# Martinsos/edlib

Hardware: NVIDIA H100
Metric: GCUPS (higher is better)
Workload: dtype u32

## Files before the change

__graft_entry__.py:

```python
import os
import subprocess
import sys

REPO = os.path.dirname(os.path.abspath(__file__))
sys.path.insert(0, REPO)


def build():
    subprocess.run(["make", "-C", os.path.join(REPO, "edlib_b200", "csrc")], check=True)
    subprocess.run(["make", "-C", os.path.join(REPO, "oracle"), "liboracle.so"], check=True)
    subprocess.run(["make", "-C", os.path.join(REPO, "oracle"), "ref"], check=True)
    subprocess.run(["make", "-C", os.path.join(REPO, "tests", "emul")], check=True)
    subprocess.run(["make", "-C", os.path.join(REPO, "tests", "kernel_probe")], check=True)
    subprocess.run(["make", "-C", os.path.join(REPO, "oracle"), "reftests"], check=True)
    subprocess.run(["make", "-C", os.path.join(REPO, "oracle"), "pybinding"], check=True)
    import edlib_b200
    import ctypes
    ctypes.CDLL(os.path.join(REPO, "edlib_b200", "lib", "libedlib_b200.so"))


def smoke():
    sys.path.insert(0, os.path.join(REPO, "tests"))
    from edlib_b200 import workloads
    from edlib_b200._ffi import EdlibLib, product_path
    lib = EdlibLib(product_path(), has_batch=True)
    assert lib.lib.edlibB200Available() == 1, "no CUDA device / kernels: the product has no CPU path"
    oracle = EdlibLib(os.path.join(REPO, "oracle", "liboracle.so"), prefix="oracle")
    target, reads = workloads.reads_vs_target(num_reads=512, read_len=150, target_len=100_000, seed=3)
# ... 16 lines not shown
```

edlib_b200/csrc/eb_common.h:

```cpp
#pragma once
#include <stdint.h>

#if defined(__CUDACC__)
#define EB_HD __host__ __device__ __forceinline__
#define EB_D __device__ __forceinline__
#else
#define EB_HD inline
#define EB_D inline
#endif

namespace eb {

struct U2 { uint32_t x, y; };

constexpr int KPOS = 4;

struct Rec {
    int best;
    int cnt;
    int last;
    int rsv;
    int pos[KPOS];
};

// ... 28 lines not shown
    int ncodes;
    const uint8_t* eqtab;
    int chunks;
    int chunkLen;
    int halo;
    Rec* recs;
    Ovf* ovf;
    int* ovfCount;
    int ovfCap;
    int prefixLen;
    int rangeMode;
};

struct K1WParams {
    const uint8_t* tcodes;
    const uint8_t* qcodes;
    const uint64_t* qoff;
    const int* qlen;
    const int* readList;
    const int* kInit;
    const int* winStart;
    const int* winLen;
    const int* trackFrom;
    int numReads;
    const int* countPtr;
    int checkAfter;
    int ncodes;
    const uint8_t* eqtab;
    WinRec* recs;
    Ovf* ovf;
    int* ovfCount;
    int ovfCap;
};

struct LJob {
    uint64_t qOff;
    uint64_t tOff;
    uint64_t matOff;
    int m, n;
    int kInit;
    int trackFrom;
};
struct LParams {
// ... 43 lines not shown
    U2* mat;
    int* colOut;
    Rec* recs;
    Ovf* ovf;
    int* ovfCount;
    int ovfCap;
};

struct PeqParams {
    const WJob* jobs;
    int numJobs;
    const uint8_t* qcodes;
    uint32_t* peq;
    int ncodes;
    const uint8_t* eqtab;
};

struct TbJob {
    uint64_t matOff;
    uint64_t qOff;
    uint64_t peqOff;
    uint64_t tOff;
    uint64_t outOff;
    int m, n, nWp;
    int rsv;
};
struct TbParams {
    const TbJob* jobs;
    int numJobs;
    const U2* mat;
// ... 72 lines not shown
    const int* qlen;
    const int* readList;
    int firstPair;
    const int* thr;
    int kBound, seedK;
    int numReads;
    int maxLen;
    int Ls;
    int Lidx, sigma, numKeys;
    const int* bucketStart;
    const int* positions;
    int maxBucket;
    int level;
    int spread;
    int* winPair;
    int* winK;
    int* winStart;
    int* winLen;
    int* winTf;
    int winCap;
    int* winCount;
    SeedPlan* plan;
};
struct Leftover {
    int pair;
    int excl;
    int bound;
};
enum RecState : int { REC_DONE = 100, REC_PENDING = 101 };
struct WinReduceParams {
// ... 172 lines not shown
```

edlib_b200/csrc/eb_core.h:

```cpp
#pragma once
#include <type_traits>

#include "eb_common.h"

#if defined(__CUDA_ARCH__)
#define EB_UNROLL _Pragma("unroll")
#else
#define EB_UNROLL
#endif

namespace eb {


EB_HD uint32_t funnel_l1(uint32_t lo, uint32_t hi) {
#if defined(__CUDA_ARCH__)
    return __funnelshift_l(lo, hi, 1);
#else
    return (hi << 1) | (lo >> 31);
#endif
}

EB_HD int popcount32(uint32_t v) {
#if defined(__CUDA_ARCH__)
    return __popc(v);
// ... 584 lines not shown
            EB_UNROLL
            for (int q = 0; q < 16; ++q) b.template column<false>(j + q, (cur.w[q >> 2] >> (8 * (q & 3))) & 255u);
        }
        for (; j + 15 <= hi; j += 16) {
            const Sym16 cur = v;
            if (j + 31 <= hi) v = load_sym16(tsyms + j + 16);
            EB_UNROLL
            for (int q = 0; q < 16; ++q) b.template column<true>(j + q, (cur.w[q >> 2] >> (8 * (q & 3))) & 255u);
        }
    }
    for (; j <= hi; ++j) b.template column<true>(j, tsyms[j]);
    bestIo = b.best;
    cntIo = b.cnt;
}

template <int NW, class WAcc>
EB_HD void k1w_profile(const K1WParams& p, int pair, int m, WAcc& acc) {
    for (int code = 0; code < p.ncodes; ++code) {
        acc.store_word(code, 0, ~0u);
        acc.store_word(code, 1, ~0u);
        acc.store_word(code, NW + 2, 0u);
        acc.store_word(code, NW + 3, 0u);
    }
    K1View<NW, WAcc> k1acc{acc};
    k1_build_peq<NW>(k1acc, p.qcodes + p.qoff[pair], m, MODE_HW, p.ncodes, p.eqtab);
}
template <int NW, class WAcc>
EB_HD void k1w_thread(const K1WParams& p, int slot, WAcc& acc) {
    const int pair = p.readList[slot];
    const int m = p.qlen[pair];
    WinRec* rec = p.recs + slot;
    k1w_profile<NW>(p, pair, m, acc);
    K1View<NW, WAcc> k1acc{acc};
    const int ws = p.winStart[slot], tf = p.trackFrom[slot], len = p.winLen[slot];
    const int kInit = p.kInit[slot];
    const int t = kInit - 1;
    const int hi = len - 1;
    if (t >= 0 && (hi - tf) + 2 * t + 1 <= 64) {
        const int c0 = tf - (m + t) > 0 ? tf - (m + t) : 0;
        int best = kInit, cnt = 0;
        k1b_sweep(acc, p.tcodes + ws, ws, m, 32 * NW - m, c0, tf, hi, t, p.checkAfter, best, cnt, rec, p, slot);
        rec->best = best;
        rec->cnt = cnt;
        return;
    }
    K1State<NW> st;
    k1_init<NW>(st, m, kInit);
// ... 2 lines not shown
        const int cntj = tf - j < 32 ? tf - j : 32;
        k1_columns<NW, false, false>(st, k1acc, PtrSyms{p.tcodes + ws + j}, cntj, ws + j, rec, slot, nullptr, nullptr, 0);
        if (st.up - st.down - (len - (j + cntj)) >= st.best) {
            hopeless = true;
            break;
        }
    }
    if (!hopeless)
        k1_columns<NW, false, true>(st, k1acc, PtrSyms{p.tcodes + ws + tf}, len - tf, ws + tf, rec, slot, p.ovf, p.ovfCount, p.ovfCap);
    rec->best = st.best;
    rec->cnt = st.cnt;
}

template <int NW, class WAcc>
EB_HD void k1w_hits_thread(const K1WParams& p, const HitParams& h, int slot, WAcc& acc) {
    HitSink sink;
    if (!hit_sink_open(h, slot, sink)) return;
    const int pair = p.readList[slot];
    const int m = p.qlen[pair];
    k1w_profile<NW>(p, pair, m, acc);
    K1View<NW, WAcc> k1acc{acc};
    const int ws = p.winStart[slot], tf = p.trackFrom[slot], len = p.winLen[slot];
    const int t = p.kInit[slot] - 1;
    const int hi = len - 1;
    if (t >= 0 && (hi - tf) + 2 * t + 1 <= 64) {
        const int c0 = tf - (m + t) > 0 ? tf - (m + t) : 0;
        int best = t, cnt = 0;
        k1b_sweep(acc, p.tcodes + ws, ws, m, 32 * NW - m, c0, tf, hi, t, p.checkAfter, best, cnt, &sink, p, slot);
    } else {
        K1State<NW> st;
        k1_init<NW>(st, m, t);
        bool hopeless = false;
        for (int j = 0; j < tf; j += 32) {
            const int cntj = tf - j < 32 ? tf - j : 32;
            k1_columns<NW, false, false>(st, k1acc, PtrSyms{p.tcodes + ws + j}, cntj, ws + j, &sink, slot, nullptr, nullptr, 0);
// ... 78 lines not shown
        }
        int lo = first - t, hi = last + t;
        if (lo <= prevHi) lo = prevHi + 1;
        if (lo < 0) lo = 0;
        if (hi > p.n - 1) hi = p.n - 1;
        if (lo > hi) continue;
        prevHi = hi;
        int ws = lo - (m + t);
        if (ws < 0) ws = 0;
        ws &= ~15;
        f(nW, ws, lo, hi);
        ++nW;
    }
    return nW;
}
EB_HD void seed_window_store(const SeedPlanParams& p, int w, int pair, int t, int ws, int lo, int hi) {
    p.winPair[w] = pair;
    p.winK[w] = t + 1;
    p.winStart[w] = ws;
    p.winLen[w] = hi - ws + 1;
    p.winTf[w] = lo - ws;
}

struct CoopSerial {
    static constexpr int W = 1;
    static EB_HD int lane() { return 0; }
    static EB_HD int width() { return 1; }
    static EB_HD void sync() {}
    static EB_HD bool any(bool v) { return v; }
    static EB_HD int add_shared(int* p, int v) {
        const int old = *p;
        *p = old + v;
// ... 132 lines not shown
                }
            }
        }
    }
    int myWs = 0, myLo = 0, myHi = 0;
    const int nW = seed_windows(p, E, c, m, t, [&](int w, int ws, int lo, int hi) {
        if (w == lane) {
            myWs = ws;
            myLo = lo;
            myHi = hi;
        }
    });
    const int base = C::reserve(p.winCount, nW);
    if (nW > 0) {
        if (base + nW <= p.winCap) {
            if (lane < nW) seed_window_store(p, base + lane, pair, t, myWs, myLo, myHi);
            if (nW > W)
                seed_windows(p, E, c, m, t, [&](int w, int ws, int lo, int hi) {
                    if (w >= W && w % W == lane) seed_window_store(p, base + w, pair, t, ws, lo, hi);
                });
            pl.first = base;
            pl.count = nW;
            pl.state = SEED_WINDOWS;
        } else {
            pl.state = SEED_SATURATED;
        }
    }
    if (live && lane == 0) p.plan[slot] = pl;
}

EB_HD void win_reduce_read(const WinReduceParams& p, int slot) {
    const SeedPlan pl = p.plan[slot];
    Rec out;
    out.best = 0x7fffffff;
// ... 818 lines not shown
EB_HD void dump_chunk_scores(int* out, const uint32_t* Pv, const uint32_t* Mv, uint32_t sb,
                             int chunkIdx, int off, int m) {
    int score = (int)sb;
    for (int i = R - 1; i >= 0; --i) {
        for (int b = 31; b >= 0; --b) {
            const long long g = ((long long)chunkIdx * R + i) * 32 + b;
            const long long r = g - off;
            if (r >= 0 && r < m) out[r] = score;
            score -= (int)((Pv[i] >> b) & 1u);
            score += (int)((Mv[i] >> b) & 1u);
        }
    }
}

EB_HD void peq_build_words(const PeqParams& p, int jobIdx, int firstWord, int wordStride) {
    const WJob J = p.jobs[jobIdx];
    const int off = 32 * J.nWp - J.m;
    const uint32_t padBit = (J.mode == MODE_HW) ? 1u : 0u;
    const uint8_t* q = p.qcodes + J.qOff;
    const bool rev = (J.flags & WF_QREV) != 0;
    uint32_t* dst = p.peq + J.peqOff;
    for (int w = firstWord; w < J.nWp; w += wordStride) {
        for (int code = 0; code < p.ncodes; ++code) {
            uint32_t bits = 0;
            for (int b = 0; b < 32; ++b) {
                const int g = w * 32 + b;
                uint32_t bit;
                if (g < off) {
                    bit = padBit;
                } else {
// ... 153 lines not shown
```

edlib_b200/csrc/eb_engine.cpp:

```cpp
#include "eb_engine_internal.h"

#include <sched.h>

namespace eb {

static int env_int(const char* name, int dflt) {
    const char* s = getenv(name);
    return (s && *s) ? atoi(s) : dflt;
}

static std::vector<int> parse_cpulist(const char* path) {
    std::vector<int> cpus;
    FILE* f = fopen(path, "r");
    if (!f) return cpus;
    char buf[4096];
    if (fgets(buf, sizeof(buf), f)) {
        for (char* tok = strtok(buf, ",\n"); tok; tok = strtok(nullptr, ",\n")) {
            int a = 0, b = 0;
            const int got = sscanf(tok, "%d-%d", &a, &b);
            if (got == 1) b = a;
            if (got >= 1)
                for (int c = a; c <= b && c < 4096; ++c) cpus.push_back(c);
        }
    }
// ... 44 lines not shown
    filterMinLevelReads = env_int("EDLIB_B200_FILTER_MIN_LEVEL_READS", filterMinLevelReads);
    tinySweepReads = env_int("EDLIB_B200_TINY_SWEEP_READS", tinySweepReads);
    filterSeedLevels = std::min(SEED_LEVELS, env_int("EDLIB_B200_FILTER_SEED_LEVELS", filterSeedLevels));
    filterMaxWindows = env_int("EDLIB_B200_FILTER_MAX_WINDOWS", filterMaxWindows);
    filterMinLen = env_int("EDLIB_B200_FILTER_MIN_LEN", filterMinLen);
    filterSpread = env_int("EDLIB_B200_FILTER_SPREAD", filterSpread);
    filterMinTarget = env_int("EDLIB_B200_FILTER_MIN_TARGET", filterMinTarget);
    filterSkipRepeats = env_int("EDLIB_B200_FILTER_SKIP_REPEATS", filterSkipRepeats);
    bandKernel = env_int("EDLIB_B200_BAND_KERNEL", bandKernel);
    collapseEqualities = env_int("EDLIB_B200_COLLAPSE_EQUALITIES", collapseEqualities);
    directUpload = env_int("EDLIB_B200_DIRECT_UPLOAD", directUpload);
    streamSlices = std::max(1, env_int("EDLIB_B200_STREAM_SLICES", streamSlices));
    directMinBytes = (size_t)env_int("EDLIB_B200_DIRECT_MIN_KB", (int)(directMinBytes >> 10)) << 10;
    deviceStage = env_int("EDLIB_B200_DEVICE_STAGE", deviceStage);
    windowCheckAfter = env_int("EDLIB_B200_WINDOW_CHECK", windowCheckAfter);
    longHwMinTarget = env_int("EDLIB_B200_LONG_HW_MIN_TARGET", longHwMinTarget);
    longSeedMaxK = env_int("EDLIB_B200_LONG_SEED_MAX_K", longSeedMaxK);
    devSliceReads = std::max(64, env_int("EDLIB_B200_SLICE_READS", devSliceReads));
    streamMinPairs = env_int("EDLIB_B200_STREAM_MIN_PAIRS", streamMinPairs);
    const int sliceMb = env_int("EDLIB_B200_SLICE_MB", 0);
    if (sliceMb > 0) sliceBytes = (size_t)sliceMb << 20;
    if (sliceMb > 0) pathSliceBytes = (size_t)sliceMb << 20;
}

static int code_map(const uint32_t (&present)[8], uint8_t (&map)[256], int other) {
    int ncodes = 0;
    for (int b = 0; b < 256; ++b) ncodes += (present[b >> 5] >> (b & 31)) & 1u;
    int next = 0;
    for (int b = 0; b < 256; ++b) {
        if (present[b >> 5] >> (b & 31) & 1u) map[b] = (uint8_t)next++;
// ... 1124 lines not shown
```

edlib_b200/csrc/eb_engine.h:

```cpp
#pragma once
#include <stddef.h>
#include <stdint.h>

#include <map>
#include <stdexcept>
#include <string>
#include <utility>
#include <vector>

#include "../../include/edlib.h"
#include "../../include/edlib_b200.h"
#include "eb_common.h"

namespace eb {

struct Backend {
    virtual ~Backend() {}
    virtual void* alloc(size_t bytes) = 0;
    virtual void free(void* p) = 0;
    virtual void* alloc_host(size_t bytes) = 0;
    virtual void free_host(void* p) = 0;
    virtual bool host_pinned(const void* , size_t ) { return false; }
    virtual void h2d(void* dst, const void* src, size_t bytes) = 0;
    virtual void d2h(void* dst, const void* src, size_t bytes) = 0;
// ... 61 lines not shown

struct EngineTunables {
    int k1MinGroup = 32;
    int k1MinChunk = 1024;
    int ovfCap = 1 << 20;
    size_t sliceBytes = 1ull << 30;
    size_t pathSliceBytes = 8ull << 30;
    size_t packParallelBytes = 32u << 20;
    int deviceStage = 1;
    int devSliceReads = 1 << 20;
    int streamSlices = 8;
    int streamMinPairs = 32768;
    int longHwMinTarget = 65536;
    int longSeedMaxK = 1024;
    int windowCheckAfter = 48;
    int filterSeedK = 20;
    int filterSeedBucket = 128;
    int filterSeedLevels = 4;
    int tinySweepReads = 8;
    int filterMinLevelReads = 64;
    int filterSeedSlack = 4;
    int filterK1 = 8;
    int filterK0 = 16;
    int filterMinLen = 96;
    int filterSpread = 1024;
    int filterMaxWindows = 32;
    int filterMinTarget = 65536;
    size_t directMinBytes = 1u << 20;
    int directUpload = 1;
    int collapseEqualities = 1;
// ... 64 lines not shown
```

edlib_b200/csrc/eb_engine_internal.h:

```cpp
#pragma once
#include "eb_engine.h"

#include <stdio.h>
#include <stdlib.h>
#include <string.h>

#include <algorithm>
#include <cmath>
#include <exception>
#include <functional>
#include <atomic>
#include <condition_variable>
#include <mutex>
#include <chrono>
#include <map>
#include <memory>
#include <stdexcept>
#include <thread>
#include <unordered_map>

namespace eb {


struct Trace {
// ... 394 lines not shown
    DevBuf<uint32_t> dMask;
    DevBuf<uint8_t> dMap;
    int ncodes = 0;
};

struct TargetHandle {
    const char* ptr = nullptr;
    int n = 0;
    size_t bytes = 0;
    DevBuf<uint8_t> codes;
    TargetCodes tc;
    SeedIndex idx;
};

struct WinJobs {
    DevBuf<int> pair, k, start, len, tf;
    int cap = 0;
    int* count = nullptr;
    void alloc(Backend* be, int n) {
        pair.alloc(be, n);
        k.alloc(be, n);
        start.alloc(be, n);
        len.alloc(be, n);
        tf.alloc(be, n);
        cap = n;
    }
};
struct WinRecords {
    WinRec* recs;
    Ovf* ovf;
    int* ovfCount;
    int ovfCap;
};

constexpr int DEV_EXTRA_SLACK = 16384;
inline long long dev_slice_pool(long long count) { return 4 * count + count / 4 + DEV_EXTRA_SLACK; }
struct DevSlice {
    int t = 0, nw = 0;
    int firstPair = -1;
    size_t listOff = 0;
    int count = 0;
// ... 61 lines not shown
            for (size_t i = lo; i < hi; ++i) {
                best[i] = -1;
                cnt[i] = 0;
                posStart[i] = -1;
                posLen[i] = 0;
            }
        });
    }

    SeedIndex* seedIdx = nullptr;
    SeedIndex ownIdx;
    bool seed_index(int t);

    SeedPlanParams seed_plan_params(const Target& tg, int level) const;
    int plan_windows(SeedPlanParams sp, WinJobs& jobs, int cap, bool hostCount);
    void sweep_windows(const Target& tg, int nw, const WinJobs& jobs, int numJobs, const WinRecords& out);
    void reduce_windows(WinReduceParams rp, const SeedPlan* plan, int numReads, const WinRecords& wr, Rec* out, int* extra,
                        int* extraCount, int extraCap);

    struct LaneGroup {
        int t, nw;
        const std::vector<int>& list;
        const Target& tg;
        int n;
        std::vector<int> bound;
        std::vector<int> excl;
        std::vector<int> direct;
        std::vector<uint8_t> repeat;
    };

    void lane_geometry(const LaneGroup& c, int g, int nwL, int& chunks, int& chunkLen, bool perChunkRecs);
// ... 69 lines not shown
```

edlib_b200/csrc/eb_kernels.cu:

```cuda
#include <cuda_runtime.h>
#include <ctype.h>
#include <stdio.h>
#include <sys/syscall.h>
#include <unistd.h>
#include <stdlib.h>
#include <string.h>

#include <algorithm>
#include <mutex>
#include <stdexcept>
#include <string>
#include <vector>

#include "eb_core.h"
#include "eb_dispatch.h"
#include "eb_engine.h"

namespace eb {

#if defined(__CUDA_ARCH__)
#define EB_DEV(expr, fallback) expr
#else
#define EB_DEV(expr, fallback) fallback
#endif
// ... 251 lines not shown
    }
};

template <int NW, int THREADS>
__global__ void __launch_bounds__(THREADS) k1w_kernel(const K1WParams p) {
    extern __shared__ __align__(128) unsigned char smem[];
    const int slot = blockIdx.x * THREADS + threadIdx.x;
    int numJobs = p.numReads;
    if (p.countPtr) numJobs = min(numJobs, *p.countPtr);
    if (slot >= numJobs) return;
    SmemWordAcc<THREADS, NW + 4> acc;
    acc.base = smem_u32(smem) + 4u * threadIdx.x;
    k1w_thread<NW>(p, slot, acc);
}

template <int NW, int THREADS>
__global__ void __launch_bounds__(THREADS) k1w_hits_kernel(const K1WParams p, const HitParams h) {
    extern __shared__ __align__(128) unsigned char smem[];
    const int slot = blockIdx.x * THREADS + threadIdx.x;
    if (slot >= p.numReads) return;
    SmemWordAcc<THREADS, NW + 4> acc;
    acc.base = smem_u32(smem) + 4u * threadIdx.x;
    k1w_hits_thread<NW>(p, h, slot, acc);
}

template <int NW>
__global__ void k1_hits_kernel(const K1Params p, const HitParams h) {
    extern __shared__ __align__(128) unsigned char smem[];
    const int slot = blockIdx.x * blockDim.x + threadIdx.x;
    if (slot >= p.numReads) return;
// ... 630 lines not shown
        while (block > 32 && perThread * block > 96 * 1024) block >>= 1;
        const size_t smem = perThread * block;
        if (smem > (size_t)maxSmemOptin) throw std::runtime_error("lane kernel: alphabet too large for shared memory");
        with_nw(nw, [&](auto w) {
            with_lane_class(mode, rev, store, [&](auto c) {
                using C = decltype(c);
                launch("lane", lane_kernel<decltype(w)::value, C::MODE, C::REV, C::STORE>, (p.numJobs + block - 1) / block, block, smem, p);
            });
        });
    }
    void launch_res(const ResParams& p) override {
        if (p.numItems <= 0) return;
        launch("res", res_kernel, (p.numItems + 255) / 256, 256, 0, p);
    }
    void launch_peq(const PeqParams& p) override {
        launch("peq", peq_kernel, (p.numJobs + W_WARPS - 1) / W_WARPS, W_WARPS * 32, 0, p);
    }
    void launch_w(const WParams& p, int R) override {
        with_r(R, [&](auto r) { launch("w", w_kernel<decltype(r)::value>, (p.numJobs + W_WARPS - 1) / W_WARPS, W_WARPS * 32, 0, p); });
    }
    static size_t band_smem(int NB, int ncodes) { return (size_t)ncodes * (4 * NB + BAND_SLACK) * 4 * BAND_THREADS; }
    int band_max_blocks(int ncodes) override {
        int nb = 0;
        while (nb < 8 && band_smem(nb + 1, ncodes) <= (size_t)110 * 1024) ++nb;
        return nb;
    }
    void launch_band(const WParams& p, int NB, int ncodes) override {
        with_nb(NB, [&](auto nb) {
            launch("band", band_kernel<decltype(nb)::value>, (p.numJobs + BAND_THREADS - 1) / BAND_THREADS, BAND_THREADS, band_smem(NB, ncodes), p,
                   ncodes);
// ... 112 lines not shown
```

edlib_b200/csrc/eb_pass_lane.cpp:

```cpp
#include "eb_engine_internal.h"

namespace eb {

bool build_seed_index(Backend* be, const EngineTunables& tun, SeedIndex& sx, const uint8_t* tcodes, int n, int ncodes) {
    sx.n = n;
    sx.ok = false;
    const int sigma = std::max(2, ncodes);
    int L0 = 4;
    double v = std::pow((double)sigma, 4);
    while (v < (double)tun.filterSeedSlack * (double)n && L0 < 32) {
        v *= sigma;
        ++L0;
    }
    if (n < 4 * L0) return false;
    const int step = (sigma * sigma <= 32) ? 2 : 1;
    for (int level = 0; level < SEED_LEVELS; ++level) {
        const int L = level < 3 ? L0 - step * level : L0 - step * 2 - (level - 2);
        const bool useful = L >= 4 && (level == 0 || (double)n / std::pow((double)sigma, L) <= 128.0);
        sx.Ls[level] = useful ? L : 0;
    }
    int Lidx = 1;
    long long keys = sigma;
    const long long maxKeys = std::min<long long>(std::max<long long>(2LL * n, 4096), 1LL << 28);
    while (Lidx < 16 && keys * sigma <= maxKeys) {
// ... 53 lines not shown
    sp.Lidx = sx.Lidx;
    sp.sigma = sx.sigma;
    sp.numKeys = sx.numKeys;
    sp.bucketStart = sx.bucketStart.p;
    sp.positions = sx.positions.p;
    sp.maxBucket = std::min(tun.filterSeedBucket << (1 + 3 * level), 8192);
    sp.level = level;
    sp.spread = tun.filterSpread;
    return sp;
}

int Pass::plan_windows(SeedPlanParams sp, WinJobs& jobs, int cap, bool hostCount) {
    for (;;) {
        jobs.alloc(be, cap);
        sp.winPair = jobs.pair.p;
        sp.winK = jobs.k.p;
        sp.winStart = jobs.start.p;
        sp.winLen = jobs.len.p;
        sp.winTf = jobs.tf.p;
        sp.winCap = cap;
        sp.winCount = jobs.count;
        be->launch_seed_plan(sp);
        if (!hostCount) return -1;
        int V = 0;
        be->d2h(&V, jobs.count, sizeof(int));
        stats.d2hBytes += 4;
        if (V <= cap) return V;
        cap = V;
        be->zero(jobs.count, sizeof(int));
    }
}

K1WParams Pass::window_params(const Target& tg, const WinJobs& jobs, int numJobs) const {
    K1WParams wp;
    memset(&wp, 0, sizeof(wp));
    wp.tcodes = p->dSeq.p + tg.off;
    wp.qcodes = p->dSeq.p;
    wp.qoff = p->dQoff.p;
    wp.qlen = p->dQlen.p;
    wp.readList = jobs.pair.p;
    wp.kInit = jobs.k.p;
    wp.winStart = jobs.start.p;
    wp.winLen = jobs.len.p;
    wp.trackFrom = jobs.tf.p;
    wp.numReads = numJobs < 0 ? jobs.cap : numJobs;
    wp.countPtr = numJobs < 0 ? jobs.count : nullptr;
    wp.checkAfter = tun.windowCheckAfter;
    wp.ncodes = p->ncodes;
    wp.eqtab = p->hasEq ? p->dEqtab.p : nullptr;
    return wp;
}

void Pass::sweep_windows(const Target& tg, int nw, const WinJobs& jobs, int numJobs, const WinRecords& out) {
    K1WParams wp = window_params(tg, jobs, numJobs);
    wp.recs = out.recs;
    wp.ovf = out.ovf;
    wp.ovfCount = out.ovfCount;
    wp.ovfCap = out.ovfCap;
    be->launch_k1w(wp, nw);
}

void Pass::reduce_windows(WinReduceParams rp, const SeedPlan* plan, int numReads, const WinRecords& wr, Rec* out, int* extra,
                          int* extraCount, int extraCap) {
    rp.plan = plan;
    rp.winRecs = wr.recs;
    rp.numReads = numReads;
    rp.out = out;
    rp.extra = extra;
    rp.extraCount = extraCount;
    rp.extraCap = extraCap;
    rp.ovf = wr.ovf;
    rp.ovfCount = wr.ovfCount;
    rp.ovfCap = wr.ovfCap;
    be->launch_win_reduce(rp);
// ... 290 lines not shown
    sp.maxLen = 32 * nw;
    sp.plan = dPlan.p;
    WinJobs jobs;
    jobs.count = dCount.p;
    be->zero(dCount.p, sizeof(int));
    const int V = plan_windows(sp, jobs, cap, true);
    perRead = (int)(((long long)V + g - 1) / g);
    stats.filterWindows += V;
    trace.mark("filter: seeds planned");
    DevBuf<WinRec> dWinRecs(be, (size_t)std::max(V, 1));
    const int ovfCap = (int)std::min<long long>((long long)V / 8 + 65536, 1 << 24);
    DevBuf<Ovf> dOvf(be, (size_t)ovfCap);
    DevBuf<int> dOvfCount(be, 1);
    be->zero(dOvfCount.p, sizeof(int));
    const WinRecords wr{dWinRecs.p, dOvf.p, dOvfCount.p, ovfCap};
    if (V > 0) sweep_windows(tg, nw, jobs, V, wr);
    int nSat = 0, nLong = 0;
    window_outcomes(c, in, thr.p, dPlan.p, wr, next, nSat, nLong);
    if (trace.on) {
        int nOvf = 0;
        dOvfCount.download(&nOvf, 1);
        fprintf(stderr, "[edlib_b200] filter seed stage %d, L=%d: %d reads, %d windows (%d listed end columns), %d saturated, %d long lists, %zu to the next stage\n",
                level, L, g, V, nOvf, nSat, nLong, next.size());
    }
}

void Pass::prefix_stage(LaneGroup& c, int P, int K0, const std::vector<int>& in, std::vector<int>& next) {
    const std::vector<int>& list = c.list;
    const Target& tg = c.tg;
    const int n = c.n;
    const int nw = c.nw;
// ... 18 lines not shown
    lane_sweep(c, cand, thr, P / 32, chunksA, chunkLenA, (int)std::min<long long>(16LL * g + 4096, 1LL << 28), P, 1, none, ranges);
    trace.mark("filter: prefix sweep");
    std::vector<int> start(g + 1, 0);
    std::vector<char> saturated(g, 0);
    for (const Ovf& o : ranges) {
        if (o.score < 0) saturated[o.rec] = 1;
        else start[o.rec + 1]++;
    }
    for (int i = 0; i < g; ++i) start[i + 1] += start[i];
    std::vector<std::pair<int, int>> rg(start[g]);
    {
        std::vector<int> fill(start.begin(), start.end() - 1);
        for (const Ovf& o : ranges)
            if (o.score >= 0) rg[fill[o.rec]++] = std::make_pair(o.score, o.pos);
    }
    std::vector<int> vPair, vK, vWs, vLen, vTf;
    std::vector<SeedPlan> plan(g);
    for (int i = 0; i < g; ++i) {
        const int s = cand[i];
        const int pair = list[s], m = p->qlen[pair], t = thr[i];
        const int w0 = (int)vPair.size();
        plan[i] = SeedPlan{w0, 0, SEED_NONE, t};
        if (saturated[i]) {
            plan[i].state = SEED_SATURATED;
            continue;
        }
        std::sort(rg.begin() + start[i], rg.begin() + start[i + 1]);
        long long prevHi = -1;
        for (int a = start[i]; a < start[i + 1];) {
            const int first = rg[a].first;
            int last = rg[a].second;
            int b = a + 1;
            while (b < start[i + 1] && rg[b].first - last <= K1_RANGE_GAP && rg[b].second - first <= tun.filterSpread) {
                last = std::max(last, rg[b].second);
                ++b;
            }
            a = b;
            long long lo = (long long)first + (m - P) - t;
            long long hi = (long long)last + (m - P) + t;
            if (lo <= prevHi) lo = prevHi + 1;
            if (lo < 0) lo = 0;
            if (hi > n - 1) hi = n - 1;
            if (lo > hi) continue;
            prevHi = hi;
            const long long ws = std::max<long long>(0, lo - (long long)(m + t)) & ~15LL;
            vPair.push_back(pair);
            vK.push_back(t + 1);
            vWs.push_back((int)ws);
            vLen.push_back((int)(hi - ws + 1));
            vTf.push_back((int)(lo - ws));
        }
        const int windows = (int)vPair.size() - w0;
        if (windows > tun.filterMaxWindows) {
            vPair.resize(w0);
            vK.resize(w0);
            vWs.resize(w0);
            vLen.resize(w0);
            vTf.resize(w0);
            plan[i].state = SEED_SATURATED;
        } else if (windows > 0) {
            plan[i].count = windows;
            plan[i].state = SEED_WINDOWS;
        }
    }
    trace.mark("filter: windows planned");
    const int V = (int)vPair.size();
    stats.filterWindows += V;
    DevBuf<SeedPlan> dPlan(be, g);
    dPlan.upload(plan.data(), g);
    DevBuf<WinRec> dRecs(be, V);
    const int ovfCap = (int)std::min<long long>((long long)V / 8 + 65536, 1 << 24);
    DevBuf<Ovf> dOvf(be, (size_t)ovfCap);
    DevBuf<int> dOvfCount(be, 1);
    be->zero(dOvfCount.p, sizeof(int));
    const WinRecords wr{dRecs.p, dOvf.p, dOvfCount.p, ovfCap};
    WinJobs jobs;
    if (V > 0) {
        jobs.alloc(be, V);
        jobs.pair.upload(vPair.data(), V);
        jobs.k.upload(vK.data(), V);
        jobs.start.upload(vWs.data(), V);
        jobs.len.upload(vLen.data(), V);
        jobs.tf.upload(vTf.data(), V);
        sweep_windows(tg, nw, jobs, V, wr);
    }
    int nSat = 0, nLong = 0;
    window_outcomes(c, cand, thr.data(), dPlan.p, wr, next, nSat, nLong);
    if (trace.on) {
        int sat = 0;
        for (char x : saturated) sat += x;
        fprintf(stderr, "[edlib_b200] filter stage P=%d: %d reads, %zu ranges, %d saturated, %d windows, %zu to the next stage\n",
                P, g, rg.size(), sat, V, next.size());
    }
}

void Pass::plain_sweep(LaneGroup& c) {
    const std::vector<int>& list = c.list;
    const std::vector<int>& direct = c.direct;
    if (direct.empty()) return;
// ... 141 lines not shown
    DevBuf<SeedPlan> dPlan(be, count);
    DevBuf<WinRec> dWinRecs(be, cap);
    DevBuf<Rec> dOut(be, count);
    DevBuf<int> dExtra(be, extraCap), dCnt32(be, (size_t)count + 1), dCtr(be, 3);
    be->zero(dCtr.p, 3 * sizeof(int));
    SeedPlanParams sp = seed_plan_params(tg, 0);
    sp.readList = dList;
    sp.firstPair = sl.firstPair;
    sp.numReads = count;
    sp.maxLen = 32 * nw;
    sp.plan = dPlan.p;
    WinJobs jobs;
    jobs.count = dCtr.p;
    plan_windows(sp, jobs, cap, false);
    const WinRecords wr{dWinRecs.p, dOvf.p, dCtr.p + 2, ovfCap};
    sweep_windows(tg, nw, jobs, -1, wr);
    WinReduceParams rp{};
    rp.leftover = dLeft.p;
    rp.leftoverCount = dLeftCount.p;
    rp.readList = dList;
    rp.firstPair = sl.firstPair;
    rp.qlen = p->dQlen.p;
    rp.kBound = k;
    rp.strands = p->strands;
    reduce_windows(rp, dPlan.p, count, wr, dOut.p, dExtra.p, dCtr.p + 1, extraCap);
    FinParams fp;
    memset(&fp, 0, sizeof(fp));
    fp.recs = dOut.p;
    fp.extra = dExtra.p;
    fp.readList = dList;
    fp.firstPair = sl.firstPair;
// ... 155 lines not shown
        sp.plan = r.dPlan.p;
        r.jobs.count = r.dWinCount.p;
        const int perRead = r.level == 0 ? 8 : r.level == 1 ? 96 : r.level == 2 ? 400 : 1500;
        r.numJobs = plan_windows(sp, r.jobs, (int)std::min<long long>((long long)g * perRead + 4096, 1LL << 28), true);
        std::vector<SeedPlan> plan((size_t)g);
        be->d2h(plan.data(), r.dPlan.p, (size_t)g * sizeof(SeedPlan));
        stats.d2hBytes += (long long)g * (long long)sizeof(SeedPlan);
        stats.filterWindows += r.numJobs;
        for (int s = 0; s < g; ++s) {
            if (plan[(size_t)s].state == SEED_SATURATED) full[r.nw].push_back(r.pairs[(size_t)s]);
            else stats.filterDecided++;
        }
        r.dCount.alloc(be, (size_t)std::max(r.numJobs, 1));
        if (r.numJobs > 0) {
            const HitParams h{r.dCount.p, nullptr, nullptr, nullptr, nullptr};
            be->launch_k1w_hits(window_params(tg, r.jobs, r.numJobs), h, r.nw);
        }
        HitPlaceParams hp;
        memset(&hp, 0, sizeof(hp));
        hp.plan = r.dPlan.p;
        hp.numReads = g;
        hp.readList = r.dList.p;
        hp.count = r.dCount.p;
        hp.pairCount = dPairCount.p;
        be->launch_hits_total(hp);
    }
    trace.mark("hits: seed windows counted");
    K1Params kp;
    memset(&kp, 0, sizeof(kp));
    kp.tcodes = p->dSeq.p + tg.off;
    kp.n = n;
// ... 87 lines not shown
        r.dRoom.alloc(be, (size_t)r.numJobs);
        HitPlaceParams hp;
        memset(&hp, 0, sizeof(hp));
        hp.plan = ri < seedRuns ? r.dPlan.p : nullptr;
        hp.chunks = r.chunks;
        hp.numReads = g;
        hp.readList = r.dList.p;
        hp.count = r.dCount.p;
        hp.pairBase = dBase.p;
        hp.pairStored = dStored.p;
        hp.at = r.dAt.p;
        hp.room = r.dRoom.p;
        be->launch_hits_place(hp);
        const HitParams h{nullptr, r.dAt.p, r.dRoom.p, dCols.p, dScores.p};
        if (ri < seedRuns) {
            be->launch_k1w_hits(window_params(tg, r.jobs, r.numJobs), h, r.nw);
        } else {
            kp.readList = r.dList.p;
            kp.kInit = r.dK.p;
            kp.numReads = g;
            kp.chunks = r.chunks;
            kp.chunkLen = r.chunkLen;
            kp.halo = 64 * r.nw;
            be->launch_k1_hits(kp, h, r.nw);
        }
    }
    dCols.download(out->columns, (size_t)S);
    dScores.download(out->scores, (size_t)S);
    stats.d2hBytes += 8 * S;
    trace.mark("hits: filled");
    if (task != EDLIB_TASK_DISTANCE) hit_alignments(task, S, stored, dBase.p, dCols.p, dScores.p, outAln);
// ... 148 lines not shown
```

edlib_b200/csrc/eb_wrunner.cpp:

```cpp
#include "eb_engine_internal.h"

namespace eb {

WPlan plan_w(int m, int n, int mode, int kBound) {
    WPlan pl;
    const int nW = ceil_div(m, 32);
    pl.slide = false;
    pl.dhi = 0;
    pl.height = 0;
    if (nW <= 32) {
        pl.R = 1;
        pl.nWp = nW;
        return pl;
    }
    pl.nWp = (int)round_up((size_t)nW, 8);
    if (mode == MODE_NW && kBound >= 0) {
        const int d = n - m;
        const int ad = d < 0 ? -d : d;
        const long long h = ((long long)kBound - ad) / 2;
        const long long dlo = std::min(0, d) - h, dhi = std::max(0, d) + h;
        const long long height = dhi - dlo + 1;
        for (int R = 1; R <= 8; R *= 2) {
            if (height + 32LL * R <= 1024LL * R && 64 * R <= nW) {
                pl.R = R;
// ... 81 lines not shown
            wj.m = t.m;
            wj.n = t.n;
            wj.nWp = ceil_div(t.m, 32);
            wj.mode = t.mode;
            wj.flags = t.flags;
            wj.kInit = t.kInit;
            wj.dhi = t.dhi;
            wj.rec = s;
            wj.peqOff = peqWords;
            peqWords += (uint64_t)p->ncodes * wj.nWp;
        }
        DevBuf<WJob> dJobs(be, (size_t)J);
        dJobs.upload(jobs.p, (size_t)J);
        DevBuf<uint32_t> dPeq(be, peqWords);
        DevBuf<Rec> dRecs(be, (size_t)J);
        PeqParams pp{dJobs.p, J, p->dSeq.p, dPeq.p, p->ncodes, p->hasEq ? p->dEqtab.p : nullptr};
        be->launch_peq(pp);
        WParams wp{dJobs.p, J, p->dSeq.p, p->dSeq.p, dPeq.p, nullptr, nullptr, nullptr, dRecs.p, nullptr, nullptr, 0};
        be->launch_band(wp, NB, p->ncodes);
        if (getenv("EDLIB_B200_TRACE")) fprintf(stderr, "[edlib_b200] band kernel: %d sweeps, window of %d words\n", J, 4 * NB);
        HostBuf<Rec> recs(be, (size_t)J);
        dRecs.download(recs.p, (size_t)J);
        eng->stats.d2hBytes += (long long)J * (long long)sizeof(Rec);
        for (int s = 0; s < J; ++s) {
            WTask& t = tasks[idx[i + s]];
            t.rec = recs[s];
            t.extra.clear();
        }
        i = j;
    }
}
// ... 154 lines not shown
            hbytes += 2 * (uint64_t)t.n;
        }
    }
    DevBuf<WJob> dJobs(be, J);
    dJobs.upload(jobs.data(), J);
    DevBuf<uint32_t> dPeq(be, peqWords);
    DevBuf<U2> dMat(be, matEntries);
    DevBuf<int> dCol(be, colInts);
    DevBuf<uint8_t> dH(be, hbytes);
    DevBuf<Rec> dRecs(be, J);
    be->zero(dRecs.p, (size_t)J * sizeof(Rec));
    DevBuf<Ovf> dOvf(be, (size_t)std::max(ovfCap, 1));
    DevBuf<int> dOvfCount(be, 1);
    be->zero(dOvfCount.p, sizeof(int));
    if (colInts) be->fill(dCol.p, 0x3f, (size_t)colInts * sizeof(int));
    PeqParams pp{dJobs.p, J, p->dSeq.p, dPeq.p, p->ncodes, p->hasEq ? p->dEqtab.p : nullptr};
    be->launch_peq(pp);
    WParams wp{dJobs.p, J, p->dSeq.p, p->dSeq.p, dPeq.p, dH.p, dMat.p, dCol.p, dRecs.p, dOvf.p, dOvfCount.p, ovfCap};
    be->launch_w(wp, R);
    if (!tb.empty()) traceback(tasks, tb, tbTask, dMat.p, dPeq.p);

    std::vector<Rec> recs(J);
    dRecs.download(recs.data(), J);
    int ovfCount = 0;
    dOvfCount.download(&ovfCount, 1);
    eng->stats.d2hBytes += (long long)J * (long long)sizeof(Rec) + 4;
    for (int s = 0; s < J; ++s) tasks[slice[s]].rec = recs[s];
    if (ovfCap > 0) {
        if (ovfCount > ovfCap) throw std::runtime_error("internal: end-location list larger than counted");
        std::vector<Ovf> ov(ovfCount);
        if (ovfCount) dOvf.download(ov.data(), ovfCount);
// ... 80 lines not shown
```

Before: 88.32 million.

## Precompute per-read query profiles once and share across window sweep jobs

Instead of each window job rebuilding the query's match-bit profile from raw query bytes, a separate kernel builds one profile per read, in pieces bounded by a configurable byte budget. Window sweep threads then copy it from global memory with vector loads. This removes the repeated profile construction when a read has many windows. In exchange it adds an extra kernel launch per piece, a profile buffer, and a device-side upload of the candidate read list. The profile builder uses SWAR byte matching and funnel-shifted word loads.

```diff
diff --git a/__graft_entry__.py b/__graft_entry__.py
--- a/__graft_entry__.py
+++ b/__graft_entry__.py
@@ -12,6 +12,7 @@
     subprocess.run(["make", "-C", os.path.join(REPO, "oracle"), "ref"], check=True)
     subprocess.run(["make", "-C", os.path.join(REPO, "tests", "emul")], check=True)
     subprocess.run(["make", "-C", os.path.join(REPO, "tests", "kernel_probe")], check=True)
+    subprocess.run(["make", "-C", os.path.join(REPO, "tests", "profile_probe")], check=True)
     subprocess.run(["make", "-C", os.path.join(REPO, "oracle"), "reftests"], check=True)
     subprocess.run(["make", "-C", os.path.join(REPO, "oracle"), "pybinding"], check=True)
     import edlib_b200
diff --git a/edlib_b200/csrc/eb_common.h b/edlib_b200/csrc/eb_common.h
--- a/edlib_b200/csrc/eb_common.h
+++ b/edlib_b200/csrc/eb_common.h
@@ -66,10 +66,11 @@
 
 struct K1WParams {
     const uint8_t* tcodes;
-    const uint8_t* qcodes;
-    const uint64_t* qoff;
-    const int* qlen;
-    const int* readList;
+    const int* qlen;
+    const int* readList;
+    const int* jobRead;
+    const uint32_t* prof;
+    int profStride, profFirst, profRows;
     const int* kInit;
     const int* winStart;
     const int* winLen;
@@ -78,7 +79,6 @@
     const int* countPtr;
     int checkAfter;
     int ncodes;
-    const uint8_t* eqtab;
     WinRec* recs;
     Ovf* ovf;
     int* ovfCount;
@@ -152,6 +152,13 @@
     uint32_t* peq;
     int ncodes;
     const uint8_t* eqtab;
+    const uint64_t* qoff;
+    const int* qlen;
+    const int* readList;
+    int firstPair;
+    int first;
+    int nw;
+    int stride;
 };
 
 struct TbJob {
@@ -254,6 +261,7 @@
     int level;
     int spread;
     int* winPair;
+    int* winRead;
     int* winK;
     int* winStart;
     int* winLen;
diff --git a/edlib_b200/csrc/eb_core.h b/edlib_b200/csrc/eb_core.h
--- a/edlib_b200/csrc/eb_core.h
+++ b/edlib_b200/csrc/eb_core.h
@@ -622,23 +622,92 @@
     cntIo = b.cnt;
 }
 
+EB_HD uint32_t zero_bytes4(uint32_t v) {
+    const uint32_t z = ~(((v & 0x7f7f7f7fu) + 0x7f7f7f7fu) | v) & 0x80808080u;
+    return ((z >> 7) * 0x10204080u) >> 28;
+}
+EB_HD void load_rows32(const uint8_t* q, int r0, uint32_t (&x)[8]) {
+#if defined(__CUDA_ARCH__)
+    const uintptr_t first = (uintptr_t)q + (r0 > 0 ? r0 : 0), last = (uintptr_t)q + r0 + 31, at = (uintptr_t)q + r0;
+    const uintptr_t base = at & ~(uintptr_t)3;
+    uint32_t v[9];
+    EB_UNROLL
+    for (int k = 0; k < 9; ++k) {
+        const uintptr_t a = base + 4 * k;
+        v[k] = (a + 3 >= first && a <= last) ? __ldg(reinterpret_cast<const uint32_t*>(a)) : 0u;
+    }
+    const int sh = 8 * (int)(at & 3);
+    EB_UNROLL
+    for (int k = 0; k < 8; ++k) x[k] = __funnelshift_r(v[k], v[k + 1], sh);
+#else
+    for (int k = 0; k < 8; ++k) {
+        x[k] = 0;
+        for (int b = 0; b < 4; ++b) {
+            const int r = r0 + 4 * k + b;
+            if (r >= 0) x[k] |= (uint32_t)q[r] << (8 * b);
+        }
+    }
+#endif
+}
+EB_HD void read_profile_word(const PeqParams& p, int r, int w) {
+    const int at = p.first + r;
+    const int pair = p.readList ? p.readList[at] : p.firstPair + at;
+    const int m = p.qlen[pair];
+    const int off = 32 * p.nw - m;
+    const uint32_t pad = ~init_pv_word(w, off);
+    uint32_t* out = p.peq + (size_t)r * p.stride + w;
+    uint32_t x[8] = {0, 0, 0, 0, 0, 0, 0, 0};
+    if (pad != ~0u) load_rows32(p.qcodes + p.qoff[pair], 32 * w - off, x);
+    for (int code = 0; code < p.ncodes; ++code) {
+        uint32_t bits = 0;
+        if (!p.eqtab) {
+            const uint32_t cc = (uint32_t)code * 0x01010101u;
+            EB_UNROLL
+            for (int k = 0; k < 8; ++k) bits |= zero_bytes4(x[k] ^ cc) << (4 * k);
+        } else {
+            for (int b = 0; b < 32; ++b) {
+                const uint32_t qc = (x[b >> 2] >> (8 * (b & 3))) & 255u;
+                if (qc < (uint32_t)p.ncodes && p.eqtab[qc * p.ncodes + code]) bits |= 1u << b;
+            }
+        }
+        out[(size_t)code * p.nw] = bits | pad;
+    }
+}
+
 template <int NW, class WAcc>
-EB_HD void k1w_profile(const K1WParams& p, int pair, int m, WAcc& acc) {
+EB_HD void k1w_profile(const K1WParams& p, int row, WAcc& acc) {
     for (int code = 0; code < p.ncodes; ++code) {
         acc.store_word(code, 0, ~0u);
         acc.store_word(code, 1, ~0u);
         acc.store_word(code, NW + 2, 0u);
         acc.store_word(code, NW + 3, 0u);
     }
-    K1View<NW, WAcc> k1acc{acc};
-    k1_build_peq<NW>(k1acc, p.qcodes + p.qoff[pair], m, MODE_HW, p.ncodes, p.eqtab);
+    const uint32_t* src = p.prof + (size_t)row * p.profStride;
+    const int words = p.ncodes * NW;
+    for (int i0 = 0; i0 < words; i0 += 16) {
+        Sym16 v[4];
+        EB_UNROLL
+        for (int j = 0; j < 4; ++j)
+            if (i0 + 4 * j < words) v[j] = load_sym16(reinterpret_cast<const uint8_t*>(src + i0 + 4 * j));
+        EB_UNROLL
+        for (int e = 0; e < 16; ++e) {
+            const int i = i0 + e;
+            if (i < words) acc.store_word(i / NW, i % NW + 2, v[e >> 2].w[e & 3]);
+        }
+    }
+}
+EB_HD int k1w_row(const K1WParams& p, int slot) {
+    const int row = p.jobRead[slot] - p.profFirst;
+    return row >= 0 && row < p.profRows ? row : -1;
 }
 template <int NW, class WAcc>
 EB_HD void k1w_thread(const K1WParams& p, int slot, WAcc& acc) {
+    const int row = k1w_row(p, slot);
+    if (row < 0) return;
     const int pair = p.readList[slot];
     const int m = p.qlen[pair];
     WinRec* rec = p.recs + slot;
-    k1w_profile<NW>(p, pair, m, acc);
+    k1w_profile<NW>(p, row, acc);
     K1View<NW, WAcc> k1acc{acc};
     const int ws = p.winStart[slot], tf = p.trackFrom[slot], len = p.winLen[slot];
     const int kInit = p.kInit[slot];
@@ -671,11 +740,12 @@
 
 template <int NW, class WAcc>
 EB_HD void k1w_hits_thread(const K1WParams& p, const HitParams& h, int slot, WAcc& acc) {
+    const int row = k1w_row(p, slot);
     HitSink sink;
-    if (!hit_sink_open(h, slot, sink)) return;
+    if (row < 0 || !hit_sink_open(h, slot, sink)) return;
     const int pair = p.readList[slot];
     const int m = p.qlen[pair];
-    k1w_profile<NW>(p, pair, m, acc);
+    k1w_profile<NW>(p, row, acc);
     K1View<NW, WAcc> k1acc{acc};
     const int ws = p.winStart[slot], tf = p.trackFrom[slot], len = p.winLen[slot];
     const int t = p.kInit[slot] - 1;
@@ -784,8 +854,9 @@
     }
     return nW;
 }
-EB_HD void seed_window_store(const SeedPlanParams& p, int w, int pair, int t, int ws, int lo, int hi) {
+EB_HD void seed_window_store(const SeedPlanParams& p, int w, int slot, int pair, int t, int ws, int lo, int hi) {
     p.winPair[w] = pair;
+    if (p.winRead) p.winRead[w] = slot;
     p.winK[w] = t + 1;
     p.winStart[w] = ws;
     p.winLen[w] = hi - ws + 1;
@@ -948,10 +1019,10 @@
     const int base = C::reserve(p.winCount, nW);
     if (nW > 0) {
         if (base + nW <= p.winCap) {
-            if (lane < nW) seed_window_store(p, base + lane, pair, t, myWs, myLo, myHi);
+            if (lane < nW) seed_window_store(p, base + lane, slot, pair, t, myWs, myLo, myHi);
             if (nW > W)
                 seed_windows(p, E, c, m, t, [&](int w, int ws, int lo, int hi) {
-                    if (w >= W && w % W == lane) seed_window_store(p, base + w, pair, t, ws, lo, hi);
+                    if (w >= W && w % W == lane) seed_window_store(p, base + w, slot, pair, t, ws, lo, hi);
                 });
             pl.first = base;
             pl.count = nW;
@@ -1800,6 +1871,10 @@
 }
 
 EB_HD void peq_build_words(const PeqParams& p, int jobIdx, int firstWord, int wordStride) {
+    if (!p.jobs) {
+        for (int w = firstWord; w < p.nw; w += wordStride) read_profile_word(p, jobIdx, w);
+        return;
+    }
     const WJob J = p.jobs[jobIdx];
     const int off = 32 * J.nWp - J.m;
     const uint32_t padBit = (J.mode == MODE_HW) ? 1u : 0u;
diff --git a/edlib_b200/csrc/eb_engine.cpp b/edlib_b200/csrc/eb_engine.cpp
--- a/edlib_b200/csrc/eb_engine.cpp
+++ b/edlib_b200/csrc/eb_engine.cpp
@@ -82,6 +82,8 @@
     directMinBytes = (size_t)env_int("EDLIB_B200_DIRECT_MIN_KB", (int)(directMinBytes >> 10)) << 10;
     deviceStage = env_int("EDLIB_B200_DEVICE_STAGE", deviceStage);
     windowCheckAfter = env_int("EDLIB_B200_WINDOW_CHECK", windowCheckAfter);
+    const int profileKb = env_int("EDLIB_B200_PROFILE_KB", 0);
+    if (profileKb > 0) profileBytes = (size_t)profileKb << 10;
     longHwMinTarget = env_int("EDLIB_B200_LONG_HW_MIN_TARGET", longHwMinTarget);
     longSeedMaxK = env_int("EDLIB_B200_LONG_SEED_MAX_K", longSeedMaxK);
     devSliceReads = std::max(64, env_int("EDLIB_B200_SLICE_READS", devSliceReads));
diff --git a/edlib_b200/csrc/eb_engine.h b/edlib_b200/csrc/eb_engine.h
--- a/edlib_b200/csrc/eb_engine.h
+++ b/edlib_b200/csrc/eb_engine.h
@@ -99,6 +99,7 @@
     int longHwMinTarget = 65536;
     int longSeedMaxK = 1024;
     int windowCheckAfter = 48;
+    size_t profileBytes = 256u << 20;
     int filterSeedK = 20;
     int filterSeedBucket = 128;
     int filterSeedLevels = 4;
diff --git a/edlib_b200/csrc/eb_engine_internal.h b/edlib_b200/csrc/eb_engine_internal.h
--- a/edlib_b200/csrc/eb_engine_internal.h
+++ b/edlib_b200/csrc/eb_engine_internal.h
@@ -432,17 +432,22 @@
 };
 
 struct WinJobs {
-    DevBuf<int> pair, k, start, len, tf;
+    DevBuf<int> pair, read, k, start, len, tf;
     int cap = 0;
     int* count = nullptr;
     void alloc(Backend* be, int n) {
         pair.alloc(be, n);
+        read.alloc(be, n);
         k.alloc(be, n);
         start.alloc(be, n);
         len.alloc(be, n);
         tf.alloc(be, n);
         cap = n;
     }
+};
+struct StageReads {
+    const int* list;
+    int firstPair, count;
 };
 struct WinRecords {
     WinRec* recs;
@@ -534,7 +539,8 @@
 
     SeedPlanParams seed_plan_params(const Target& tg, int level) const;
     int plan_windows(SeedPlanParams sp, WinJobs& jobs, int cap, bool hostCount);
-    void sweep_windows(const Target& tg, int nw, const WinJobs& jobs, int numJobs, const WinRecords& out);
+    void sweep_windows(const Target& tg, int nw, const StageReads& reads, const WinJobs& jobs, int numJobs, const WinRecords& out);
+    void with_read_profiles(const StageReads& reads, int nw, K1WParams wp, const std::function<void(const K1WParams&)>& launch);
     void reduce_windows(WinReduceParams rp, const SeedPlan* plan, int numReads, const WinRecords& wr, Rec* out, int* extra,
                         int* extraCount, int extraCap);
 
diff --git a/edlib_b200/csrc/eb_kernels.cu b/edlib_b200/csrc/eb_kernels.cu
--- a/edlib_b200/csrc/eb_kernels.cu
+++ b/edlib_b200/csrc/eb_kernels.cu
@@ -289,6 +289,12 @@
     k1w_thread<NW>(p, slot, acc);
 }
 
+__global__ void read_profile_kernel(const PeqParams p) {
+    const int i = blockIdx.x * blockDim.x + threadIdx.x;
+    const int r = i / p.nw;
+    if (r < p.numJobs) read_profile_word(p, r, i - r * p.nw);
+}
+
 template <int NW, int THREADS>
 __global__ void __launch_bounds__(THREADS) k1w_hits_kernel(const K1WParams p, const HitParams h) {
     extern __shared__ __align__(128) unsigned char smem[];
@@ -949,6 +955,11 @@
         launch("res", res_kernel, (p.numItems + 255) / 256, 256, 0, p);
     }
     void launch_peq(const PeqParams& p) override {
+        if (!p.jobs) {
+            const int items = p.numJobs * p.nw;
+            if (items > 0) launch("read_profile", read_profile_kernel, (items + 255) / 256, 256, 0, p);
+            return;
+        }
         launch("peq", peq_kernel, (p.numJobs + W_WARPS - 1) / W_WARPS, W_WARPS * 32, 0, p);
     }
     void launch_w(const WParams& p, int R) override {
diff --git a/edlib_b200/csrc/eb_pass_lane.cpp b/edlib_b200/csrc/eb_pass_lane.cpp
--- a/edlib_b200/csrc/eb_pass_lane.cpp
+++ b/edlib_b200/csrc/eb_pass_lane.cpp
@@ -91,6 +91,7 @@
     for (;;) {
         jobs.alloc(be, cap);
         sp.winPair = jobs.pair.p;
+        sp.winRead = jobs.read.p;
         sp.winK = jobs.k.p;
         sp.winStart = jobs.start.p;
         sp.winLen = jobs.len.p;
@@ -112,10 +113,9 @@
     K1WParams wp;
     memset(&wp, 0, sizeof(wp));
     wp.tcodes = p->dSeq.p + tg.off;
-    wp.qcodes = p->dSeq.p;
-    wp.qoff = p->dQoff.p;
     wp.qlen = p->dQlen.p;
     wp.readList = jobs.pair.p;
+    wp.jobRead = jobs.read.p;
     wp.kInit = jobs.k.p;
     wp.winStart = jobs.start.p;
     wp.winLen = jobs.len.p;
@@ -124,17 +124,43 @@
     wp.countPtr = numJobs < 0 ? jobs.count : nullptr;
     wp.checkAfter = tun.windowCheckAfter;
     wp.ncodes = p->ncodes;
-    wp.eqtab = p->hasEq ? p->dEqtab.p : nullptr;
     return wp;
 }
 
-void Pass::sweep_windows(const Target& tg, int nw, const WinJobs& jobs, int numJobs, const WinRecords& out) {
+void Pass::with_read_profiles(const StageReads& reads, int nw, K1WParams wp, const std::function<void(const K1WParams&)>& launch) {
+    PeqParams pp;
+    memset(&pp, 0, sizeof(pp));
+    pp.qcodes = p->dSeq.p;
+    pp.ncodes = p->ncodes;
+    pp.eqtab = p->hasEq ? p->dEqtab.p : nullptr;
+    pp.qoff = p->dQoff.p;
+    pp.qlen = p->dQlen.p;
+    pp.readList = reads.list;
+    pp.firstPair = reads.firstPair;
+    pp.nw = nw;
+    pp.stride = (int)round_up((size_t)p->ncodes * nw, 4);
+    const int piece = (int)std::max<long long>(1, std::min<long long>(reads.count, (long long)tun.profileBytes / (4LL * pp.stride)));
+    DevBuf<uint32_t> prof(be, (size_t)piece * pp.stride);
+    pp.peq = prof.p;
+    wp.prof = prof.p;
+    wp.profStride = pp.stride;
+    for (int first = 0; first < reads.count; first += piece) {
+        pp.first = first;
+        pp.numJobs = std::min(piece, reads.count - first);
+        be->launch_peq(pp);
+        wp.profFirst = first;
+        wp.profRows = pp.numJobs;
+        launch(wp);
+    }
+}
+
+void Pass::sweep_windows(const Target& tg, int nw, const StageReads& reads, const WinJobs& jobs, int numJobs, const WinRecords& out) {
     K1WParams wp = window_params(tg, jobs, numJobs);
     wp.recs = out.recs;
     wp.ovf = out.ovf;
     wp.ovfCount = out.ovfCount;
     wp.ovfCap = out.ovfCap;
-    be->launch_k1w(wp, nw);
+    with_read_profiles(reads, nw, wp, [&](const K1WParams& w) { be->launch_k1w(w, nw); });
 }
 
 void Pass::reduce_windows(WinReduceParams rp, const SeedPlan* plan, int numReads, const WinRecords& wr, Rec* out, int* extra,
@@ -455,7 +481,7 @@
     DevBuf<int> dOvfCount(be, 1);
     be->zero(dOvfCount.p, sizeof(int));
     const WinRecords wr{dWinRecs.p, dOvf.p, dOvfCount.p, ovfCap};
-    if (V > 0) sweep_windows(tg, nw, jobs, V, wr);
+    if (V > 0) sweep_windows(tg, nw, StageReads{dList.p, 0, g}, jobs, V, wr);
     int nSat = 0, nLong = 0;
     window_outcomes(c, in, thr.p, dPlan.p, wr, next, nSat, nLong);
     if (trace.on) {
@@ -504,7 +530,7 @@
         for (const Ovf& o : ranges)
             if (o.score >= 0) rg[fill[o.rec]++] = std::make_pair(o.score, o.pos);
     }
-    std::vector<int> vPair, vK, vWs, vLen, vTf;
+    std::vector<int> vPair, vRead, vK, vWs, vLen, vTf;
     std::vector<SeedPlan> plan(g);
     for (int i = 0; i < g; ++i) {
         const int s = cand[i];
@@ -535,6 +561,7 @@
             prevHi = hi;
             const long long ws = std::max<long long>(0, lo - (long long)(m + t)) & ~15LL;
             vPair.push_back(pair);
+            vRead.push_back(i);
             vK.push_back(t + 1);
             vWs.push_back((int)ws);
             vLen.push_back((int)(hi - ws + 1));
@@ -543,6 +570,7 @@
         const int windows = (int)vPair.size() - w0;
         if (windows > tun.filterMaxWindows) {
             vPair.resize(w0);
+            vRead.resize(w0);
             vK.resize(w0);
             vWs.resize(w0);
             vLen.resize(w0);
@@ -568,11 +596,16 @@
     if (V > 0) {
         jobs.alloc(be, V);
         jobs.pair.upload(vPair.data(), V);
+        jobs.read.upload(vRead.data(), V);
         jobs.k.upload(vK.data(), V);
         jobs.start.upload(vWs.data(), V);
         jobs.len.upload(vLen.data(), V);
         jobs.tf.upload(vTf.data(), V);
-        sweep_windows(tg, nw, jobs, V, wr);
+        std::vector<int> candPairs(g);
+        for (int i = 0; i < g; ++i) candPairs[i] = list[cand[i]];
+        DevBuf<int> dCand(be, g);
+        dCand.upload(candPairs.data(), g);
+        sweep_windows(tg, nw, StageReads{dCand.p, 0, g}, jobs, V, wr);
     }
     int nSat = 0, nLong = 0;
     window_outcomes(c, cand, thr.data(), dPlan.p, wr, next, nSat, nLong);
@@ -744,7 +777,7 @@
     jobs.count = dCtr.p;
     plan_windows(sp, jobs, cap, false);
     const WinRecords wr{dWinRecs.p, dOvf.p, dCtr.p + 2, ovfCap};
-    sweep_windows(tg, nw, jobs, -1, wr);
+    sweep_windows(tg, nw, StageReads{dList, sl.firstPair, count}, jobs, -1, wr);
     WinReduceParams rp{};
     rp.leftover = dLeft.p;
     rp.leftoverCount = dLeftCount.p;
@@ -930,7 +963,8 @@
         r.dCount.alloc(be, (size_t)std::max(r.numJobs, 1));
         if (r.numJobs > 0) {
             const HitParams h{r.dCount.p, nullptr, nullptr, nullptr, nullptr};
-            be->launch_k1w_hits(window_params(tg, r.jobs, r.numJobs), h, r.nw);
+            with_read_profiles(StageReads{r.dList.p, 0, g}, r.nw, window_params(tg, r.jobs, r.numJobs),
+                               [&](const K1WParams& wp) { be->launch_k1w_hits(wp, h, r.nw); });
         }
         HitPlaceParams hp;
         memset(&hp, 0, sizeof(hp));
@@ -1048,7 +1082,8 @@
         be->launch_hits_place(hp);
         const HitParams h{nullptr, r.dAt.p, r.dRoom.p, dCols.p, dScores.p};
         if (ri < seedRuns) {
-            be->launch_k1w_hits(window_params(tg, r.jobs, r.numJobs), h, r.nw);
+            with_read_profiles(StageReads{r.dList.p, 0, g}, r.nw, window_params(tg, r.jobs, r.numJobs),
+                               [&](const K1WParams& wp) { be->launch_k1w_hits(wp, h, r.nw); });
         } else {
             kp.readList = r.dList.p;
             kp.kInit = r.dK.p;
diff --git a/edlib_b200/csrc/eb_wrunner.cpp b/edlib_b200/csrc/eb_wrunner.cpp
--- a/edlib_b200/csrc/eb_wrunner.cpp
+++ b/edlib_b200/csrc/eb_wrunner.cpp
@@ -119,7 +119,13 @@
         dJobs.upload(jobs.p, (size_t)J);
         DevBuf<uint32_t> dPeq(be, peqWords);
         DevBuf<Rec> dRecs(be, (size_t)J);
-        PeqParams pp{dJobs.p, J, p->dSeq.p, dPeq.p, p->ncodes, p->hasEq ? p->dEqtab.p : nullptr};
+        PeqParams pp{};
+        pp.jobs = dJobs.p;
+        pp.numJobs = J;
+        pp.qcodes = p->dSeq.p;
+        pp.peq = dPeq.p;
+        pp.ncodes = p->ncodes;
+        pp.eqtab = p->hasEq ? p->dEqtab.p : nullptr;
         be->launch_peq(pp);
         WParams wp{dJobs.p, J, p->dSeq.p, p->dSeq.p, dPeq.p, nullptr, nullptr, nullptr, dRecs.p, nullptr, nullptr, 0};
         be->launch_band(wp, NB, p->ncodes);
@@ -304,7 +310,13 @@
     DevBuf<int> dOvfCount(be, 1);
     be->zero(dOvfCount.p, sizeof(int));
     if (colInts) be->fill(dCol.p, 0x3f, (size_t)colInts * sizeof(int));
-    PeqParams pp{dJobs.p, J, p->dSeq.p, dPeq.p, p->ncodes, p->hasEq ? p->dEqtab.p : nullptr};
+    PeqParams pp{};
+    pp.jobs = dJobs.p;
+    pp.numJobs = J;
+    pp.qcodes = p->dSeq.p;
+    pp.peq = dPeq.p;
+    pp.ncodes = p->ncodes;
+    pp.eqtab = p->hasEq ? p->dEqtab.p : nullptr;
     be->launch_peq(pp);
     WParams wp{dJobs.p, J, p->dSeq.p, p->dSeq.p, dPeq.p, dH.p, dMat.p, dCol.p, dRecs.p, dOvf.p, dOvfCount.p, ovfCap};
     be->launch_w(wp, R);
```

After: 91.96 million (median of 6 runs). 1.04x the previous value.
